# Ladme/groan_rs

Hardware: AMD Instinct MI355X
Metric: frames/sec RMSD-fit, 1e6 atoms triclinic, 1/2/4/8 GPUs; HBM GB/s vs peak (higher is better)
Workload: dtype f32 (fp64 accumulators)

## Files before the change

### groan_rs_amd/csrc/gr_api.hip

```cpp
#include <hip/hip_runtime.h>

#include <cmath>
#include <cstdio>
#include <cstdlib>
#include <cstring>
#include <map>
#include <string>
#include <vector>

#include "../../include/groan_hip.h"
#include "gr_container.h"
#include "gr_kernels.h"
#include "gr_hot.h"
#include "gr_resident.h"
#include "gr_small.h"
#include "gr_xtc.h"
#include "gr_shape.h"
#include "gr_xtc_dev.h"
#include "gr_xtc_enc_dev.h"
#include "gr_trr.h"
#include "gr_cellgrid.h"
#include "gr_textio.h"
#include "gr_pool.h"
#include <set>
// ... 76 lines not shown
    struct Metro { uint64_t shape = 0; double free_ns = 0, T_ns = 0, best_ns = 0, fail_ns = 0; uint32_t off_for = 0, held = 0; } metro;
    uint64_t res_metro_period_ns = 0, res_last_turn_ns = 0, res_late_permille = 0, res_sclk_mhz = 0;
    int wall_khz = 100000;
    uint32_t res_max_wgs = 0;
    int res_test_no_start = 0;
    uint32_t res_test_abort_at = 0xFFFFFFFFu;
    uint32_t res_skip = 0, res_backoff = 0;
    uint32_t *res_progress = nullptr;
    unsigned long long *res_wgrec = nullptr; size_t res_wgrec_cap = 0;
    unsigned long long *res_rec = nullptr;
    uint32_t *res_abort = nullptr;
    uint32_t *res_words_host = nullptr;
    struct ResOut { GrFrameState st[GR_MAX_BATCH]; uint32_t words[16]; alignas(64) uint32_t seq; };
    ResOut *res_out = nullptr, *res_out_dev = nullptr;
    uint32_t res_seq = 0;
    uint32_t res_checkin = 0, res_closed = 0;
    uint32_t res_late_seen[2] = { 0, 0 };
    uint64_t res_lean_segments = 0, res_sync_fallbacks = 0;
    GrShapeSet *shape_set_dev = nullptr;
    unsigned long long *shape_mask_dev = nullptr, *shape_mask_host = nullptr; size_t shape_mask_cap = 0;
    uint32_t res_epoch = 0;
    bool res_in_use = false;
    uint64_t res_launches = 0, res_handshake_misses = 0, res_aborts = 0, res_redone_frames = 0;
    GrFrameState *state_dev = nullptr;
    GrFrameState *state_host = nullptr;
    GrFrameState *small_state = nullptr, *small_state_dev = nullptr;
    uint32_t *small_flag = nullptr, *small_flag_dev = nullptr;
    uint32_t small_seq = 0;
    uint32_t small_max = GR_SMALL_MAX_DEFAULT;
    uint64_t small_calls = 0, small_sync_fallbacks = 0;
    uint32_t *bad_dev = nullptr;
    uint32_t *bad_host = nullptr;
    float *pd_out = nullptr; size_t pd_cap = 0;
    hipEvent_t ev0 = nullptr, ev1 = nullptr;
    hipEvent_t pev[6 * GR_MAX_BATCH] = {};
    uint32_t sub_batch = 256;
    uint32_t chunks = 0;
    uint32_t fit_wgs = 0;
    int profile = 0;
    double prof_ms[4] = { 0, 0, 0, 0 };
    uint64_t prof_launches[4] = { 0, 0, 0, 0 };
    uint64_t prof_frames[4] = { 0, 0, 0, 0 };
    uint32_t n_cus = 0;
    unsigned char *xtc_host[2] = { nullptr, nullptr }, *xtc_dev[2] = { nullptr, nullptr }; size_t xtc_host_cap[2] = { 0, 0 }, xtc_dev_cap[2] = { 0, 0 };
    hipEvent_t xtc_ev[2] = { nullptr, nullptr };
    hipEvent_t xtc_unpacked[2] = { nullptr, nullptr };
// ... 237 lines not shown
    int st = busy_check(c); if (st) return st;
    Group g;
    st = group_build(c, std::move(blocks), &g); if (st) return st;
    const bool existed = c->groups.count(name) != 0;
    if (existed) group_release(c, c->groups[name]);
    c->groups[name] = g;
    c->epoch++;
    return existed ? GR_E_GROUP_EXISTS : GR_OK;
}

const Group *find_group(const gr_ctx *c, const char *name) {
    if (!name) return nullptr;
    auto it = c->groups.find(name);
    return it == c->groups.end() ? nullptr : &it->second;
}

int box_check(gr_ctx *c, uint32_t slot) {
    const int st = c->box_status[slot];
    if (st == GR_E_NO_BOX) return fail(c, GR_E_NO_BOX, "simulation box does not exist");
    if (c->strict && !c->boxes_host[slot].ortho) return fail(c, GR_E_NOT_ORTHOGONAL, "simulation box is not orthogonal");
    if (st != GR_OK) return fail(c, st, st == GR_E_ZERO_BOX ? "box length is not positive" : "box too skewed");
    return GR_OK;
}

int slot_check(gr_ctx *c, uint32_t slot, uint32_t n = 1, bool ingest = false) {
    if (!c) return GR_E_INVALID_ARG;
    if ((uint64_t)slot + n > c->n_slots || n == 0) return fail(c, GR_E_INVALID_ARG, "slot out of range");
    if (!ingest) return busy_check(c);
    if (c->in_flight && slot < c->in_flight_s0 + c->in_flight_n && c->in_flight_s0 < slot + n)
        return fail(c, GR_E_INVALID_ARG, "upload into a slot of the batch in flight: call gr_rmsd_batch_end first (or use the other half of the double buffer)");
    return GR_OK;
}

struct SlotUse {
    gr_ctx *c; uint32_t first, n;
    bool quiet = false;
    SlotUse(gr_ctx *ctx, uint32_t first_slot, uint32_t count = 1) : c(ctx), first(first_slot), n(count) {
        for (uint32_t s = first; s < first + n && s < c->n_slots; ++s)
            if (c->upload_pending[s]) { (void)hipStreamWaitEvent(c->stream, c->ev_ready[s], 0); c->upload_pending[s] = 0; }
    }
    ~SlotUse() {
        if (quiet) return;
        const uint64_t gen = ++c->done_gen;
        (void)hipEventRecord(c->ev_done_ring[gen % 64], c->stream);
        for (uint32_t s = first; s < first + n && s < c->n_slots; ++s) c->slot_gen[s] = gen;
    }
};

static hipError_t sync_ingest(gr_ctx *c) {
    hipError_t e = hipStreamSynchronize(c->copy_stream);
    if (e == hipSuccess && c->unpack_stream) e = hipStreamSynchronize(c->unpack_stream);
    return e;
}
void box_fill(gr_ctx *c, uint32_t slot, const float *box9) {
    GrBox &b = c->boxes_host[slot];
    if (!box9) {
        gr_box_setup(nullptr, &b);
        c->box_status[slot] = GR_E_NO_BOX; c->box9_set[slot] = 0;
    } else {
        const int ok = gr_box_setup(box9, &b);
        memcpy(&c->box9_host[9 * (size_t)slot], box9, 9 * sizeof(float));
        c->box9_set[slot] = 1;
        if (!ok) c->box_status[slot] = GR_E_ZERO_BOX;
        else if (b.ncand > GR_MAX_CAND) c->box_status[slot] = GR_E_UNSUPPORTED_BOX;
        else c->box_status[slot] = GR_OK;
    }
}
int set_box(gr_ctx *c, uint32_t slot, const float *box9, hipStream_t on = nullptr) {
    box_fill(c, slot, box9);
    HIPCHK(c, hipMemcpyAsync(c->boxes_dev + slot, &c->boxes_host[slot], sizeof(GrBox), hipMemcpyHostToDevice, on ? on : c->stream));
    return GR_OK;
}

int set_boxes_same(gr_ctx *c, uint32_t first_slot, uint32_t n, const float *box9, hipStream_t on = nullptr) {
    if (n == 0) return GR_OK;
    float keep[9];
    if (box9) memcpy(keep, box9, sizeof keep);
    box_fill(c, first_slot, box9 ? keep : nullptr);
// ... 67 lines not shown

static int res_next_epoch(gr_ctx *c, uint32_t *epoch) {
    if (++c->res_epoch == 0u) {
        HIPCHK(c, hipStreamSynchronize(c->stream));
        if (c->res_wgrec) HIPCHK(c, hipMemset(c->res_wgrec, 0, c->res_wgrec_cap * sizeof(unsigned long long)));
        HIPCHK(c, hipMemset(c->res_rec, 0, (size_t)GR_MAX_BATCH * 16 * sizeof(unsigned long long)));
        HIPCHK(c, hipMemset(c->res_abort + 2, 0, 2 * sizeof(uint32_t)));
        c->res_epoch = 1u;
    }
    *epoch = c->res_epoch;
    return GR_OK;
}
static int res_test_no_start(gr_ctx *c, uint32_t epoch) {
    if (!c->res_test_no_start) return GR_OK;
    const unsigned long long two = 2ull | ((unsigned long long)epoch << 32);
    c->res_test_no_start = 0;
    HIPCHK(c, hipMemcpyAsync(c->res_abort + 2, &two, sizeof two, hipMemcpyHostToDevice, c->stream));
    HIPCHK(c, hipStreamSynchronize(c->stream));
    return GR_OK;
}
template <int MODE>
static int res_close(gr_ctx *c, uint32_t nb, const double *fit_partials, uint32_t nparts, double sum_w, uint32_t epoch, bool fresh, uint32_t *seq) {
    const uint32_t sq = c->res_seq + 1u;
    k_res_close<MODE><<<dim3(nb), dim3(64), 0, c->stream>>>(fit_partials, nparts, sum_w, c->state_dev, c->res_rec, epoch, fresh ? 1u : 0u, c->res_abort, c->res_closed + nb,
                                                        c->res_out_dev->st, c->res_out_dev->words, &c->res_out_dev->seq, sq);
    HIPCHK(c, hipGetLastError());
    c->res_seq = sq; c->res_closed += nb; *seq = sq;
    return GR_OK;
}
static int res_collect(gr_ctx *c, uint32_t seq, uint32_t nb, uint32_t epoch, bool *started) {
    volatile uint32_t *w = &c->res_out->seq;
    const auto t0 = std::chrono::steady_clock::now();
    for (uint32_t spins = 0; *w != seq; ++spins) {
        if ((spins & 1023u) == 1023u && std::chrono::steady_clock::now() - t0 > std::chrono::milliseconds(20)) {
            c->res_sync_fallbacks++;
            HIPCHK(c, hipStreamSynchronize(c->stream));
            if (*w != seq) return fail(c, GR_E_HIP, "the kernel behind the resident pass ended without publishing its results");
            break;
        }
    }
    std::atomic_thread_fence(std::memory_order_acquire);
    memcpy(c->state_host, c->res_out->st, (size_t)nb * sizeof(GrFrameState));
    memcpy(c->res_words_host, c->res_out->words, 12 * sizeof(uint32_t));
    for (int k = 0; k < 2; ++k) { const uint32_t v = c->res_words_host[8 + k]; c->res_words_host[8 + k] = v - c->res_late_seen[k]; c->res_late_seen[k] = v; }
    *started = c->res_words_host[2] == 1u && c->res_words_host[3] == epoch;
    if (!*started || c->res_words_host[0]) HIPCHK(c, hipStreamSynchronize(c->stream));
    return GR_OK;
// ... 227 lines not shown
    for (int k = 0; k < 6; ++k) if (c->xe_dev[k]) (void)hipFree(c->xe_dev[k]);
    for (int k = 0; k < 2; ++k) if (c->xe_host[k]) (void)hipHostFree(c->xe_host[k]);
    if (c->unpack_stream) { (void)hipStreamSynchronize(c->unpack_stream); (void)hipStreamDestroy(c->unpack_stream); }
    for (int k = 0; k < 2; ++k) {
        if (c->xtc_host[k]) (void)hipHostFree(c->xtc_host[k]);
        if (c->xtc_dev[k]) (void)hipFree(c->xtc_dev[k]);
        if (c->xtc_ev[k]) (void)hipEventDestroy(c->xtc_ev[k]);
        if (c->xtc_unpacked[k]) (void)hipEventDestroy(c->xtc_unpacked[k]);
    }
    if (c->wr_host) (void)hipHostFree(c->wr_host);
    if (c->ev0) (void)hipEventDestroy(c->ev0);
    if (c->ev1) (void)hipEventDestroy(c->ev1);
    for (int k = 0; k < 6 * GR_MAX_BATCH; ++k) if (c->pev[k]) (void)hipEventDestroy(c->pev[k]);
    for (hipEvent_t e : c->ev_ready) if (e) (void)hipEventDestroy(e);
    for (int k = 0; k < 64; ++k) if (c->ev_done_ring[k]) (void)hipEventDestroy(c->ev_done_ring[k]);
    if (c->copy_stream) (void)hipStreamDestroy(c->copy_stream);
    if (c->stream) (void)hipStreamDestroy(c->stream);
    delete c;
} catch (...) { }

const char *gr_last_error(const gr_ctx *c) { return c ? c->err.c_str() : "null context"; }
uint64_t gr_last_error_index(const gr_ctx *c) { return c ? c->err_index : 0; }
void gr_last_error_counts(const gr_ctx *c, uint64_t counts[2]) { if (c && counts) { counts[0] = c->counts[0]; counts[1] = c->counts[1]; } }
int gr_ctx_set_strict_orthogonal(gr_ctx *c, int on) { if (!c) return GR_E_INVALID_ARG; c->strict = on ? 1 : 0; return GR_OK; }
uint64_t gr_n_atoms(const gr_ctx *c) { return c ? c->n : 0; }
uint32_t gr_n_slots(const gr_ctx *c) { return c ? c->n_slots : 0; }

int gr_sync(gr_ctx *c) try {
    if (!c) return GR_E_INVALID_ARG;
    HIPCHK(c, sync_ingest(c));
    HIPCHK(c, hipStreamSynchronize(c->stream));
    return GR_OK;
} catch (...) { return gr_abi_guard(); }

int gr_set_masses(gr_ctx *c, const float *masses, uint64_t n) try {
    if (!c || !masses || n != c->n) return c ? fail(c, GR_E_INVALID_ARG, "masses: size mismatch") : GR_E_INVALID_ARG;
    { int st = busy_check(c); if (st) return st; }
    c->masses_host.assign(masses, masses + n);
    c->epoch++;
    HIPCHK(c, hipMemcpyAsync(c->masses, masses, n * sizeof(float), hipMemcpyHostToDevice, c->stream));
    HIPCHK(c, hipStreamSynchronize(c->stream));
    return GR_OK;
} catch (...) { return gr_abi_guard(); }

size_t gr_container_from_indices(const uint64_t *indices, size_t n, uint64_t n_atoms, uint64_t *os, uint64_t *oe) try {
    return grc::store(grc::from_indices(std::vector<uint64_t>(indices, indices + n), n_atoms), os, oe);
} catch (...) { return 0; }
// ... 821 lines not shown
    if (rec_words > c->res_wgrec_cap) {
        if (c->res_wgrec) (void)hipFree(c->res_wgrec);
        c->res_wgrec = nullptr; c->res_wgrec_cap = 0;
        HIPCHK(c, hipMalloc(&c->res_wgrec, rec_words * sizeof(unsigned long long)));
        HIPCHK(c, hipMemsetAsync(c->res_wgrec, 0, rec_words * sizeof(unsigned long long), S));
        c->res_wgrec_cap = rec_words;
    }
    GrResCtl ctl;
    memset(&ctl, 0, sizeof ctl);
    { const int se = res_next_epoch(c, &ctl.epoch); if (se) return se; }
    ctl.wgrec = c->res_wgrec; ctl.rec = c->res_rec; ctl.abort = c->res_abort; ctl.progress = c->res_progress; ctl.n_stream = res_stream; ctl.n_fin = n_fin;
    ctl.checkin_target = c->res_checkin + res_stream + n_fin; ctl.fresh_states = fresh_states ? 1u : 0u;
    ctl.wgs_frame = wgs; ctl.streams = streams; ctl.groups_wg = gwg;
    ctl.team_waves = resident_team_waves(wgs, streams);
    ctl.patience_ticks = (unsigned long long)c->wall_khz * 3000ull; ctl.start_ticks = (unsigned long long)c->wall_khz * 200ull;
    ctl.test_abort_frame = c->res_test_abort_at; c->res_test_abort_at = 0xFFFFFFFFu;
    ctl.metro_t16 = c->res_metro_ns >= 100 ? (uint32_t)std::min<uint64_t>(0xFFFFFFFFull, (uint64_t)c->res_metro_ns * (uint64_t)c->wall_khz * 16ull / 1000000ull) : 0u;
    ctl.metro_lead = (uint32_t)((uint64_t)c->wall_khz * 2000ull / 1000000ull);
    ctl.cen_weighted = weighted ? 1u : 0u; ctl.cen_dim_mask = (uint32_t)dim_mask;
    float *frames = c->frames; size_t stride = c->frame_stride; uint32_t slot0 = s0, nfr = nb, natoms = (uint32_t)c->n;
    const float *masses = c->masses; GrSel sel_arg = csel; const GrBox *boxes = c->boxes_dev; GrPlanDev plan; memset(&plan, 0, sizeof plan);
    GrFrameState *states = c->state_dev; double *fparts = nullptr;
    void *args[] = { &frames, &stride, &slot0, &nfr, &natoms, &masses, &sel_arg, &boxes, &plan, &states, &fparts, &ctl };
    bool ubox = true;
    for (uint32_t f = 1; f < nb && ubox; ++f) ubox = memcmp(&c->boxes_host[s0 + f], &c->boxes_host[s0], sizeof(GrBox)) == 0;
    const bool fit_last = c->res_fit_last ? c->res_fit_last == 2 : (uint64_t)res_stream * 10u >= (uint64_t)c->res_max_wgs * 9u;
    { const int sn = res_test_no_start(c, ctl.epoch); if (sn) return sn; }
    if (hipLaunchKernel(resident_center_fn(ubox, fit_last), dim3(res_stream + n_fin), dim3(GrResShape::LANES), args, GrResShape::LDS_BYTES, S) != hipSuccess) {
        (void)hipGetLastError();
        c->res_max_wgs = 0;
        return GR_OK;
    }
    c->res_checkin += res_stream + n_fin;
    uint32_t seq = 0; bool started = false;
    { const int sc = res_close<1>(c, nb, nullptr, 0u, 1.0, ctl.epoch, fresh_states, &seq); if (sc) return sc; }
    { const int sc = res_collect(c, seq, nb, ctl.epoch, &started); if (sc) return sc; }
    c->res_last_streams = streams;
    if (!started) {
        c->res_handshake_misses++;
        c->res_backoff = c->res_backoff ? std::min<uint32_t>(c->res_backoff * 2u, 1024u) : 4u;
        c->res_skip = c->res_backoff;
        return GR_OK;
    }
    c->res_backoff = 0;
    c->cen_res_launches++;
    if (fresh_states) c->res_lean_segments++;
    ran = true;
#ifdef GR_EXP_STEPTIME
// ... 215 lines not shown
int gr_ctx_stat(const gr_ctx *c, int key, uint64_t *value) {
    if (!c || !value) return GR_E_INVALID_ARG;
    switch (key) {
    case GR_STAT_N_CUS: *value = c->n_cus; return GR_OK;
    case GR_STAT_RES_MAX_WGS: *value = c->res_max_wgs; return GR_OK;
    case GR_STAT_RES_LAST_STREAMS: *value = c->res_last_streams; return GR_OK;
    case GR_STAT_RES_LAUNCHES: *value = c->res_launches; return GR_OK;
    case GR_STAT_RES_HANDSHAKE_MISSES: *value = c->res_handshake_misses; return GR_OK;
    case GR_STAT_RES_ABORTS: *value = c->res_aborts; return GR_OK;
    case GR_STAT_RES_REDONE_FRAMES: *value = c->res_redone_frames; return GR_OK;
    case GR_STAT_RMSD_FAST_FRAMES: *value = c->rmsd_fast_frames; return GR_OK;
    case GR_STAT_RMSD_EXACT_REDOS: *value = c->rmsd_exact_redos; return GR_OK;
    case GR_STAT_XTC_DEVICE_FRAMES: *value = c->xtc_dev_frames; return GR_OK;
    case GR_STAT_SMALL_CALLS: *value = c->small_calls; return GR_OK;
    case GR_STAT_SMALL_SYNC_FALLBACKS: *value = c->small_sync_fallbacks; return GR_OK;
    case GR_STAT_RES_METRO_PERIOD_NS: *value = c->res_metro_period_ns; return GR_OK;
    case GR_STAT_RES_LAST_TURN_NS: *value = c->res_last_turn_ns; return GR_OK;
    case GR_STAT_RES_LATE_PERMILLE: *value = c->res_late_permille; return GR_OK;
    case GR_STAT_RES_SCLK_MHZ: *value = c->res_sclk_mhz; return GR_OK;
    case GR_STAT_CENTER_RES_LAUNCHES: *value = c->cen_res_launches; return GR_OK;
    case GR_STAT_CENTER_RES_REDONE: *value = c->cen_res_redone; return GR_OK;
    case GR_STAT_RES_LEAN_SEGMENTS: *value = c->res_lean_segments; return GR_OK;
    case GR_STAT_RES_SYNC_FALLBACKS: *value = c->res_sync_fallbacks; return GR_OK;
    default: return GR_E_INVALID_ARG;
    }
}
int gr_ctx_set_tuning(gr_ctx *c, int key, int64_t value) try {
    if (!c) return GR_E_INVALID_ARG;
    { int st = busy_check(c); if (st) return st; }
    switch (key) {
    case GR_TUNE_SUB_BATCH: if (value < 1 || value > GR_MAX_BATCH) break; c->sub_batch = (uint32_t)value; return GR_OK;
    case GR_TUNE_CHUNKS: if (value < 0 || value > GR_MAX_CHUNKS) break; c->chunks = (uint32_t)value; return GR_OK;
    case GR_TUNE_FIT_WGS: if (value < 0 || value > 65535) break; c->fit_wgs = (uint32_t)value; return GR_OK;
    case GR_TUNE_FUSE: c->fuse = value ? 1 : 0; return GR_OK;
    case GR_TUNE_SMALL_CALLS: if (value < 0 || value > 65536) break; c->small_max = (uint32_t)value; return GR_OK;
    case GR_TUNE_TWO_PASS: c->two_pass = value ? 1 : 0; return GR_OK;
    case GR_TUNE_RESIDENT: if (value < 0 || value > 2) break; c->resident = value; return GR_OK;
    case GR_TUNE_MASKED_SELECTIONS: if (value != 0 && value != 1) break; c->masked_sel = (int)value; return GR_OK;
    case GR_TUNE_XTC_DEVICE_ENCODE: if (value != 0 && value != 1) break; c->xtc_dev_encode = (int)value; return GR_OK;
    case GR_TUNE_RMSD_FAST: if (value != 0 && value != 1) break; c->rmsd_fast = (int)value; return GR_OK;
    case GR_TUNE_RMSD_FAST_MIN: if (value < 0 || value > 0x7fffffff) break; c->rmsd_fast_min = (uint32_t)value; return GR_OK;
    case GR_TUNE_RMSD_FAST_SIGMAS: if (value < 0 || value > 1000) break; c->rmsd_fast_sigmas = (int)value; return GR_OK;
    case GR_TUNE_PAIRDIST_SYMMETRIC: if (value != 0 && value != 1) break; c->pd_sym = (int)value; return GR_OK;
    case GR_TUNE_RESIDENT_WG_GROUPS: if (value != 0 && (value < 64 || value > GR_RES_GROUPS || value % 64 != 0)) break; c->res_wg_groups = (int)value; return GR_OK;
    case GR_TUNE_RESIDENT_STREAMS: if (value < 0 || value > GR_RES_MAX_STREAMS) break; c->res_streams = (int)value; return GR_OK;
    case GR_TUNE_RESIDENT_METRO_NS: if (value < 0 || value > 1000000 || (value > 1 && value < 100)) break; c->res_metro_ns = (int)value; c->metro = gr_ctx::Metro(); return GR_OK;
// ... 15 lines not shown
    if (small_ok(c, sel)) {
        k_rmsd_small<1><<<dim3(nf), dim3(64), 0, c->stream>>>(c->frames, c->frame_stride, first_slot, c->masses, sel, c->boxes_dev, p->dev, c->state_dev, 1, nullptr, nullptr, 0u);
    } else {
        const uint32_t nch = chunks_for(sel);
        k_rmsd_accum<1><<<dim3(nch, nf), dim3(GR_WG), 0, c->stream>>>(c->frames, c->frame_stride, first_slot, c->masses, sel, c->boxes_dev, p->dev, c->state_dev, c->acc_partials);
        k_rmsd_finalize<1><<<dim3(nf), dim3(GR_WG), 0, c->stream>>>(c->acc_partials, nch, c->frames, c->frame_stride, first_slot, sel, c->boxes_dev, p->dev, c->state_dev);
    }
    if (fit) {
        const uint32_t gx = (uint32_t)std::min<uint64_t>(((c->n >> 2) + GR_WG * 4 - 1) / (GR_WG * 4) + 1, 1024);
        k_fit_pk<false><<<dim3(gx, nf), dim3(GR_WG), 0, c->stream>>>(c->frames, c->frame_stride, first_slot, (uint32_t)c->n, c->boxes_dev, p->dev, c->state_dev, c->masses, sel, nullptr);
    }
    HIPCHK(c, hipGetLastError());
    return GR_OK;
}

static int segment_begin(gr_rmsd_plan *p, uint32_t s0, uint32_t nb, int fit) {
    gr_ctx *c = p->target;
    Pending &q = p->pend;
    q = Pending();
    q.s0 = s0; q.nb = nb; q.fit = fit; q.active = true;
    SlotUse use(c, s0, nb);
    const Group *g = find_group(c, p->group.c_str());
    q.pre.assign(nb, GR_OK); q.pre_idx.assign(nb, 0); q.pre_msg.assign(nb, std::string());
    for (uint32_t f = 0; f < nb; ++f) {
        int s = box_check(c, s0 + f);
        if (s == GR_OK && !g) s = fail(c, GR_E_GROUP_NOT_FOUND, p->group);
        if (s == GR_OK && g->n == 0) s = fail(c, GR_E_EMPTY_GROUP, p->group);
        q.pre[f] = s;
        if (s != GR_OK) { q.pre_msg[f] = c->err; q.pre_idx[f] = c->err_index; }
        q.any_ok = q.any_ok || s == GR_OK;
    }
    if (!q.any_ok) return GR_OK;
    const GrSel sel = make_sel(*g);
    q.sel = sel; q.group_n = g->n; q.has_group = true;
    if (!p->resolved || p->resolved_epoch != c->epoch) {
        p->resolved_epoch = c->epoch;
        bool same = (g->n == p->n_ref);
        if (same) { size_t k = 0; for (uint64_t i : grc::expand(g->blocks)) { const float a = c->masses_host[i], b = p->w_host[k++]; if (!(a == b)) { same = false; break; } } }
        p->dev.w_is_mass = same ? 1u : 0u; p->resolved = true;
        p->span_ok = p->p_span_dev != nullptr && g->masked && g->mask_dev != nullptr && g->blocks == p->ref_blocks;
    }
    q.consistent = (g->n == p->n_ref);
    const bool fast_asked = c->two_pass && c->rmsd_fast && p->dev.w_is_mass != 0 && g->n >= c->rmsd_fast_min && ((!fit && sel.contiguous) || (sel.masked && p->span_ok));
    const bool small = q.consistent && !p->exact && small_ok(c, sel) && !fast_asked;
    if (small && nb == 1) {
        q.small = true; q.small_seq = ++c->small_seq;
        k_rmsd_small<0><<<dim3(1), dim3(64), 0, c->stream>>>(c->frames, c->frame_stride, s0, c->masses, sel, c->boxes_dev, p->dev,
                                                         c->state_dev, 0, c->small_state_dev, c->small_flag_dev, q.small_seq);
        if (fit) k_fit_pk<false><<<dim3(fit_grid(c, 1), 1), dim3(GR_WG), 0, c->stream>>>(c->frames, c->frame_stride, s0, (uint32_t)c->n, c->boxes_dev, p->dev, c->state_dev, c->masses, sel, nullptr);
        p->fit_behind_small = fit != 0;
        HIPCHK(c, hipGetLastError());
        return GR_OK;
    }
// ... 87 lines not shown
                ctl.metro_lead = (uint32_t)((uint64_t)c->wall_khz * 2000ull / 1000000ull);
            }
#ifdef GR_EXP_STEPTIME
            {
                static unsigned long long *dbg_dev = nullptr;
                if (!dbg_dev) (void)hipMalloc(&dbg_dev, (size_t)GR_MAX_CHUNKS * 8 * 4 * sizeof(unsigned long long));
                ctl.dbg = getenv("GR_STEPTIME") ? dbg_dev : nullptr;
                g_steptime_dbg = ctl.dbg;
            }
#endif
#ifdef GR_EXP_TIMELINE
            {
                static unsigned long long *tl_dev = nullptr; static size_t tl_cap = 0;
                if (nb > tl_cap) { if (tl_dev) (void)hipFree(tl_dev); tl_dev = nullptr; tl_cap = 0; if (hipMalloc(&tl_dev, (size_t)nb * 8 * sizeof(unsigned long long)) == hipSuccess) tl_cap = nb; }
                ctl.tl = getenv("GR_TIMELINE") ? tl_dev : nullptr;
                if (ctl.tl) HIPCHK(c, hipMemsetAsync(ctl.tl, 0, (size_t)nb * 8 * sizeof(unsigned long long), S));
                q.tl_dev = ctl.tl;
            }
#endif
            float *frames = c->frames; size_t stride = c->frame_stride; uint32_t slot0 = s0, nfr = nb, natoms = (uint32_t)c->n;
            const float *masses = c->masses; GrSel sel_arg = sel; const GrBox *boxes = c->boxes_dev; GrPlanDev plan = res_msk ? plan_span : p->dev;
            GrFrameState *states = c->state_dev; double *fparts = c->fit_partials;
            void *args[] = { &frames, &stride, &slot0, &nfr, &natoms, &masses, &sel_arg, &boxes, &plan, &states, &fparts, &ctl };
            bool ubox = true;
            for (uint32_t f = 1; f < nb && ubox; ++f) ubox = memcmp(&c->boxes_host[s0 + f], &c->boxes_host[s0], sizeof(GrBox)) == 0;
#ifdef GR_EXP_NO_UBOX
            ubox = false;
#endif
            const bool whole = sel.start == 0 && sel.n == c->n;
            const bool fit_last = c->res_fit_last ? c->res_fit_last == 2 : (uint64_t)res_stream * 10u >= (uint64_t)c->res_max_wgs * 9u;
            const void *fn = resident_fn(p->dev.w_is_mass != 0, ubox, whole, fit_last);
            const uint32_t lanes = GrResShape::LANES, lds = GrResShape::LDS_BYTES;
            st = res_test_no_start(c, ctl.epoch); if (st) return st;
            if (c->profile) EVREC(c, c->pev[0], true, S);
            const hipError_t le = hipLaunchKernel(fn, dim3(res_stream + n_fin), dim3(lanes), args, lds, S);
            if (le == hipSuccess) {
                if (c->profile) EVREC(c, c->pev[1], true, S);
                c->res_checkin += res_stream + n_fin;
                q.res_fresh = states_unset; q.res_epoch = ctl.epoch;
                states_unset = false;
                st = res_close<0>(c, nb, c->fit_partials, res_wgs * GrResShape::WAVES, p->dev.sw, ctl.epoch, q.res_fresh, &q.res_seq); if (st) return st;
                q.resident = true; q.res_stream = res_stream; q.res_streams = res_streams;
                q.rmsd_fast = false;
                c->res_last_streams = res_streams;
            } else {
                (void)hipGetLastError();
                c->res_max_wgs = 0;
                resident_done(c);
// ... 1311 lines not shown
```

### groan_rs_amd/csrc/gr_resident.h

```cpp
#pragma once
#include <type_traits>
#include "gr_hot.h"

struct GrResShape {
    static constexpr int LANES = 512, WAVES = LANES / 64;
#ifndef GR_RES_K
#define GR_RES_K 6
#endif
    static constexpr int K = GR_RES_K;
    static constexpr int R = 8;
    static constexpr int PARK_F4 = K * 3 * LANES;
    static constexpr int WSUM_F = R * WAVES * 32;
#ifdef GR_EXP_TIMELINE
    static constexpr int TL_BYTES = 128 * 4 * 8;
#else
    static constexpr int TL_BYTES = 0;
#endif
    static constexpr int LDS_BYTES = PARK_F4 * 16 + WSUM_F * 4 + R * WAVES * 8 + 3 * R * 4 + 2 * WAVES * 4 + TL_BYTES;
    static constexpr int REC_PER_WAVE = 256 / WAVES, LANES_PER_REC = 64 / REC_PER_WAVE, WORDS_PER_LANE = 32 / LANES_PER_REC;
};
#ifndef GR_RES_SLEEP
#define GR_RES_SLEEP 2
#endif
#ifndef GR_RES_BAL
// ... 925 lines not shown
            unsigned long long *o = reinterpret_cast<unsigned long long *>(ctl.abort + 16) + ((wg_all ? 2u : 0u) + (wave ? 1u : 0u)) * 8u;
            for (int k = 0; k < 8; ++k) o[k] = st_acc[k];
        }
#endif
        if (clk_wave) {
            const unsigned long long dc = (unsigned long long)clock64() - clk_c0, dw = (unsigned long long)wall_clock64() - clk_w0;
            gr_st_agent(ctl.abort + 10, (uint32_t)(dc >> 8)); gr_st_agent(ctl.abort + 11, (uint32_t)(dw >> 8));
        }
    }
#ifdef GR_EXP_TIMELINE
    if (tl_wg && wave == 0 && !bail) {
        for (uint32_t t = (n_turns > 128u ? n_turns - 128u : 0u) + lane; t < n_turns; t += 64u) {
            const size_t f = kf(t);
            ctl.tl[f * 8 + 0] = tls[(t & 127u) * 4u + 0u];
            ctl.tl[f * 8 + 6] = tls[(t & 127u) * 4u + 1u] | (tls[(t & 127u) * 4u + 2u] << 48);
        }
    }
#endif
}

template <int MODE>
__global__ __launch_bounds__(64) void k_res_close(const double *__restrict__ fit_partials, uint32_t nparts, double sum_w, GrFrameState *state,
                                                  const unsigned long long *__restrict__ rec, uint32_t epoch, uint32_t fresh_states, uint32_t *ctl_words,
                                                  uint32_t done_target, GrFrameState *out_states, uint32_t *out_words, uint32_t *out_seq, uint32_t seq) {
    constexpr uint32_t NW = sizeof(GrFrameState) / 4u, W_RMSD = offsetof(GrFrameState, rmsd) / 4u, W_STATUS = offsetof(GrFrameState, status) / 4u;
    static_assert(sizeof(GrFrameState) % 4u == 0 && NW <= 64u, "a frame state is exported by one wave, a word per lane");
    const uint32_t frame = blockIdx.x, lane = threadIdx.x;
    uint32_t *sw = reinterpret_cast<uint32_t *>(state + frame);
    uint32_t w = 0u;
    if (fresh_states && (uint32_t)(gr_ld_agent(rec + (size_t)frame * 16u) >> 32) != epoch) {
        GrFrameState z = {};
        z.err_index = GR_NOIDX; z.status = GR_ST_ABORTED;
        if (lane < NW) { w = reinterpret_cast<const uint32_t *>(&z)[lane]; sw[lane] = w; }
    } else if (lane < NW) w = sw[lane];
    const int status = __shfl((int)w, (int)W_STATUS, 64);
    if (MODE == 0 && status == 0) {
        double s0 = 0.0, s1 = 0.0, s2 = 0.0, s3 = 0.0;
        const double *p = fit_partials + (size_t)frame * nparts;
        uint32_t k = lane;
        for (; k + 192 < nparts; k += 256) { s0 += p[k]; s1 += p[k + 64]; s2 += p[k + 128]; s3 += p[k + 192]; }
        for (; k < nparts; k += 64) s0 += p[k];
        const double s = gr_wave_sum((s0 + s1) + (s2 + s3));
        float r = 0.0f;
        if (lane == 0) { r = (float)sqrt(fmax(s, 0.0) / sum_w); state[frame].rmsd = r; }
        r = __shfl(r, 0, 64);
        if (lane == W_RMSD) w = __float_as_uint(r);
    }
    if (lane < NW) reinterpret_cast<uint32_t *>(out_states + frame)[lane] = w;
    __threadfence_system();
    uint32_t n = 0u;
    if (lane == 0) n = __hip_atomic_fetch_add(ctl_words + 12, 1u, __ATOMIC_ACQ_REL, __HIP_MEMORY_SCOPE_AGENT) + 1u;
    n = (uint32_t)__builtin_amdgcn_readfirstlane((int)n);
    if (n != done_target) return;
    if (lane < 12u) out_words[lane] = gr_ld_agent(ctl_words + lane);
    __threadfence_system();
    if (lane == 0) __hip_atomic_store(out_seq, seq, __ATOMIC_RELEASE, __HIP_MEMORY_SCOPE_SYSTEM);
}
```

### groan_rs_amd/system.py

```python
import ctypes as C
from enum import IntEnum

import numpy as np

from . import _lib
from ._lib import (OK, E_NO_BOX, E_NOT_ORTHOGONAL, E_ZERO_BOX, E_EMPTY_GROUP, E_INCONSISTENT_GROUP,
                   E_NO_POSITION, E_NO_MASS, E_GROUP_NOT_FOUND, E_OUT_OF_RANGE, E_GROUP_EXISTS, E_INVALID_NAME, E_INVALID_BOND)


class Dimension(IntEnum):
    NONE = 0
    X = 1
    Y = 2
    Z = 3
    XY = 4
    XZ = 5
    YZ = 6
    XYZ = 7

    def is_x(self):
        return self in (Dimension.X, Dimension.XY, Dimension.XZ, Dimension.XYZ)

    def is_y(self):
        return self in (Dimension.Y, Dimension.XY, Dimension.YZ, Dimension.XYZ)
# ... 284 lines not shown
        if st == E_INCONSISTENT_GROUP:
            cnt = (C.c_uint64 * 2)()
            self._lib.gr_last_error_counts(self._ctx, cnt)
            raise RMSDError("InconsistentGroup", (msg, int(cnt[0]), int(cnt[1])), st)
        raise DeviceError(self._lib.gr_status_string(st).decode(), msg, st)

    def get_n_atoms(self):
        return self.n_atoms

    def set_masses(self, masses):
        m = np.ascontiguousarray(masses, dtype=np.float32)
        st = self._lib.gr_set_masses(self._ctx, _ptr(m), m.size)
        if st != OK:
            raise DeviceError("set_masses", self._err(st)[1], st)

    TUNE = {"sub_batch": 1, "chunks": 2, "fit_wgs": 3, "fuse": 4, "two_pass": 5, "resident": 6, "resident_groups": 7, "resident_streams": 8, "resident_fill": 9, "pairdist_symmetric": 10, "resident_wg_groups": 11, "rmsd_fast": 12, "rmsd_fast_min": 13, "rmsd_fast_sigmas": 14, "masked_selections": 15, "xtc_device_encode": 16, "small_calls": 17, "resident_metro_ns": 18, "resident_fit_last": 19, "stream_wgs_per_cu": 20, "center_resident": 21, "translate_rows": 22, "test_resident_no_start": 100, "test_resident_abort_at": 101}

    def set_tuning(self, **kw):
        for k, v in kw.items():
            st = self._lib.gr_ctx_set_tuning(self._ctx, self.TUNE[k], int(v))
            if st != OK:
                raise DeviceError("set_tuning", self._err(st)[1], st)

    STAT = {"n_cus": 1, "res_max_wgs": 2, "res_launches": 3, "res_handshake_misses": 4, "res_aborts": 5, "res_redone_frames": 6, "res_last_streams": 7, "rmsd_fast_frames": 8, "rmsd_exact_redos": 9, "xtc_device_frames": 10, "small_calls": 11, "small_sync_fallbacks": 12, "res_metro_period_ns": 13, "res_last_turn_ns": 14, "res_late_permille": 15, "res_sclk_mhz": 16, "center_res_launches": 17, "center_res_redone": 18, "res_lean_segments": 19, "res_sync_fallbacks": 20}

    def stat(self, key):
        v = C.c_uint64(0)
        st = self._lib.gr_ctx_stat(self._ctx, self.STAT[key], C.byref(v))
        if st != OK:
            raise DeviceError("stat", self._err(st)[1], st)
        return int(v.value)

    def set_center_onepass_min(self, min_atoms):
        self._lib.gr_ctx_set_center_onepass_min(self._ctx, int(min_atoms))

    def center_fallbacks(self):
        return int(self._lib.gr_center_fallbacks(self._ctx))

    def set_strict_orthogonal(self, on=True):
        self._strict_flag = bool(on)
        self._lib.gr_ctx_set_strict_orthogonal(self._ctx, int(bool(on)))

    def group_create_from_ranges(self, name, ranges):
        r = np.asarray(list(ranges), dtype=np.uint64).reshape(-1, 2)
        s, e = np.ascontiguousarray(r[:, 0]), np.ascontiguousarray(r[:, 1])
        st = self._lib.gr_group_create_from_ranges(self._ctx, name.encode(), _ptr(s), _ptr(e), r.shape[0])
        if st not in (OK, E_GROUP_EXISTS):
# ... 478 lines not shown
```

### include/groan_hip.h

```cpp
#ifndef GROAN_HIP_H
#define GROAN_HIP_H
#include <stddef.h>
#include <stdint.h>

#ifdef __cplusplus
extern "C" {
#endif

typedef struct gr_ctx gr_ctx;
typedef struct gr_rmsd_plan gr_rmsd_plan;
typedef struct gr_hbond_plan gr_hbond_plan;
typedef struct gr_gridmap gr_gridmap;
typedef struct gr_xtc gr_xtc;

enum {
    GR_OK = 0,
    GR_E_NO_BOX = 1,
    GR_E_NOT_ORTHOGONAL = 2,
    GR_E_ZERO_BOX = 3,
    GR_E_EMPTY_GROUP = 4,
    GR_E_INCONSISTENT_GROUP = 5,
    GR_E_NO_POSITION = 6,
    GR_E_NO_MASS = 7,
    GR_E_GROUP_NOT_FOUND = 8,
// ... 116 lines not shown
int gr_rmsd_fit_batch(gr_rmsd_plan *plan, uint32_t first_slot, uint32_t n_frames,
                      float *rmsd_out, int *status_out);
int gr_rmsd_batch_begin(gr_rmsd_plan *plan, uint32_t first_slot, uint32_t n_frames, int fit);
int gr_rmsd_batch_end(gr_rmsd_plan *plan, float *rmsd_out, int *status_out, float *R_out);
uint32_t gr_rmsd_plan_last_fallbacks(const gr_rmsd_plan *plan);
int gr_rmsd_plan_force_exact(gr_rmsd_plan *plan, int on);
enum { GR_TUNE_SUB_BATCH = 1, GR_TUNE_CHUNKS = 2, GR_TUNE_FIT_WGS = 3, GR_TUNE_FUSE = 4, GR_TUNE_TWO_PASS = 5, GR_TUNE_RESIDENT = 6, GR_TUNE_RESIDENT_GROUPS = 7,
       GR_TUNE_RESIDENT_STREAMS = 8, GR_TUNE_RESIDENT_FILL = 9, GR_TUNE_PAIRDIST_SYMMETRIC = 10, GR_TUNE_RESIDENT_WG_GROUPS = 11,
       GR_TUNE_RMSD_FAST = 12, GR_TUNE_RMSD_FAST_MIN = 13, GR_TUNE_RESIDENT_METRO_NS = 18, GR_TUNE_RESIDENT_FIT_LAST = 19, GR_TUNE_STREAM_WGS_PER_CU = 20, GR_TUNE_CENTER_RESIDENT = 21, GR_TUNE_TRANSLATE_ROWS = 22,
       GR_TUNE_MASKED_SELECTIONS = 15 ,
       GR_TUNE_XTC_DEVICE_ENCODE = 16 ,
       GR_TUNE_RMSD_FAST_SIGMAS = 14 ,
       GR_TUNE_SMALL_CALLS = 17 ,
       GR_TUNE_TEST_RESIDENT_NO_START = 100 ,
       GR_TUNE_TEST_RESIDENT_ABORT_AT = 101  };
int gr_ctx_set_tuning(gr_ctx *ctx, int key, int64_t value);
enum { GR_STAT_N_CUS = 1, GR_STAT_RES_MAX_WGS = 2, GR_STAT_RES_LAUNCHES = 3, GR_STAT_RES_HANDSHAKE_MISSES = 4, GR_STAT_RES_ABORTS = 5, GR_STAT_RES_REDONE_FRAMES = 6, GR_STAT_RES_LAST_STREAMS = 7,
       GR_STAT_RMSD_FAST_FRAMES = 8 ,
       GR_STAT_RMSD_EXACT_REDOS = 9 ,
       GR_STAT_XTC_DEVICE_FRAMES = 10 ,
       GR_STAT_SMALL_CALLS = 11 ,
       GR_STAT_SMALL_SYNC_FALLBACKS = 12 ,
       GR_STAT_RES_METRO_PERIOD_NS = 13, GR_STAT_RES_LAST_TURN_NS = 14, GR_STAT_RES_LATE_PERMILLE = 15, GR_STAT_RES_SCLK_MHZ = 16,
       GR_STAT_CENTER_RES_LAUNCHES = 17, GR_STAT_CENTER_RES_REDONE = 18, GR_STAT_RES_LEAN_SEGMENTS = 19, GR_STAT_RES_SYNC_FALLBACKS = 20 };
int gr_ctx_stat(const gr_ctx *ctx, int key, uint64_t *value);

enum { GR_PARSE_OK = 0, GR_PARSE_FILE_NOT_FOUND, GR_PARSE_LINE_NOT_FOUND, GR_PARSE_LINE, GR_PARSE_ATOM_LINE, GR_PARSE_BOX_LINE,
       GR_PARSE_UNSUPPORTED_BOX, GR_PARSE_INVALID_FLOAT, GR_PARSE_GROUP_NAME, GR_PARSE_INVALID_ATOM_INDEX };
typedef struct gr_structure gr_structure;
int gr_gro_read(const char *path, gr_structure **out, int *detail_code, char *detail, size_t detail_cap);
void gr_structure_free(gr_structure *s);
uint64_t gr_structure_n_atoms(const gr_structure *s);
const char *gr_structure_title(const gr_structure *s);
int gr_structure_box(const gr_structure *s, float box9[9]);
int gr_structure_positions(const gr_structure *s, float *xyz);
int gr_structure_velocities(const gr_structure *s, float *vel);
int gr_structure_atom(const gr_structure *s, uint64_t i, uint64_t *resid, uint64_t *atomid, char resname[8], char atomname[8]);
typedef struct gr_ndx gr_ndx;
int gr_ndx_read(const char *path, uint64_t n_atoms, gr_ndx **out, int *detail_code, char *detail, size_t detail_cap);
void gr_ndx_free(gr_ndx *x);
size_t gr_ndx_n_groups(const gr_ndx *x);
const char *gr_ndx_group_name(const gr_ndx *x, size_t g);
size_t gr_ndx_group_size(const gr_ndx *x, size_t g);
int gr_ndx_group_indices(const gr_ndx *x, size_t g, uint64_t *out);
int gr_ndx_install(const gr_ndx *x, gr_ctx *ctx, size_t *n_invalid_names, size_t *n_duplicate_names);

int gr_group_pairs_within(gr_ctx *ctx, uint32_t slot, const char *group1, const char *group2, float cutoff, uint64_t max_pairs,
// ... 134 lines not shown
```

Baseline: 140,800.

## Cache per-segment box prechecks and export resident frame states in one bulk copy

Adds a host-side cache keyed on a box generation counter, so the per-frame box validity checks and the uniform-box memcmp scan are skipped when the same segment is rerun with unchanged boxes. Reworks the resident close kernel so each wave writes its frame state only to device memory with an agent-scope release. The last wave then copies all states to the host-mapped output in one pass using 128-bit stores, replacing per-frame system-scope fences. This is meant to cut host CPU overhead and many system-wide fences per batch, at the cost of a serial copy done by a single wave and cache invalidation that must track every path that mutates boxes.

```diff
diff --git a/groan_rs_amd/csrc/gr_api.hip b/groan_rs_amd/csrc/gr_api.hip
--- a/groan_rs_amd/csrc/gr_api.hip
+++ b/groan_rs_amd/csrc/gr_api.hip
@@ -122,6 +122,9 @@
     uint32_t res_epoch = 0;
     bool res_in_use = false;
     uint64_t res_launches = 0, res_handshake_misses = 0, res_aborts = 0, res_redone_frames = 0;
+    uint64_t box_gen = 1;
+    struct PreCache { uint64_t gen = 0; uint32_t s0 = 0, nb = 0; bool boxes_ok = false, ubox_known = false, ubox = false; } pre_cache;
+    uint64_t precheck_cache_hits = 0;
     GrFrameState *state_dev = nullptr;
     GrFrameState *state_host = nullptr;
     GrFrameState *small_state = nullptr, *small_state_dev = nullptr;
@@ -405,6 +408,20 @@
     if (st != GR_OK) return fail(c, st, st == GR_E_ZERO_BOX ? "box length is not positive" : "box too skewed");
     return GR_OK;
 }
+static gr_ctx::PreCache &pre_cache_for(gr_ctx *c, uint32_t s0, uint32_t nb) {
+    gr_ctx::PreCache &pc = c->pre_cache;
+    if (pc.gen != c->box_gen || pc.s0 != s0 || pc.nb != nb) { pc = gr_ctx::PreCache(); pc.gen = c->box_gen; pc.s0 = s0; pc.nb = nb; }
+    return pc;
+}
+static bool segment_ubox(gr_ctx *c, uint32_t s0, uint32_t nb) {
+    gr_ctx::PreCache &pc = pre_cache_for(c, s0, nb);
+    if (!pc.ubox_known) {
+        bool ubox = true;
+        for (uint32_t f = 1; f < nb && ubox; ++f) ubox = memcmp(&c->boxes_host[s0 + f], &c->boxes_host[s0], sizeof(GrBox)) == 0;
+        pc.ubox = ubox; pc.ubox_known = true;
+    }
+    return pc.ubox;
+}
 
 int slot_check(gr_ctx *c, uint32_t slot, uint32_t n = 1, bool ingest = false) {
     if (!c) return GR_E_INVALID_ARG;
@@ -437,6 +454,7 @@
 }
 void box_fill(gr_ctx *c, uint32_t slot, const float *box9) {
     GrBox &b = c->boxes_host[slot];
+    c->box_gen++;
     if (!box9) {
         gr_box_setup(nullptr, &b);
         c->box_status[slot] = GR_E_NO_BOX; c->box9_set[slot] = 0;
@@ -550,7 +568,7 @@
 template <int MODE>
 static int res_close(gr_ctx *c, uint32_t nb, const double *fit_partials, uint32_t nparts, double sum_w, uint32_t epoch, bool fresh, uint32_t *seq) {
     const uint32_t sq = c->res_seq + 1u;
-    k_res_close<MODE><<<dim3(nb), dim3(64), 0, c->stream>>>(fit_partials, nparts, sum_w, c->state_dev, c->res_rec, epoch, fresh ? 1u : 0u, c->res_abort, c->res_closed + nb,
+    k_res_close<MODE><<<dim3(nb), dim3(64), 0, c->stream>>>(fit_partials, nparts, sum_w, c->state_dev, c->res_rec, epoch, fresh ? 1u : 0u, c->res_abort, c->res_closed + nb, nb,
                                                         c->res_out_dev->st, c->res_out_dev->words, &c->res_out_dev->seq, sq);
     HIPCHK(c, hipGetLastError());
     c->res_seq = sq; c->res_closed += nb; *seq = sq;
@@ -824,7 +842,7 @@
 const char *gr_last_error(const gr_ctx *c) { return c ? c->err.c_str() : "null context"; }
 uint64_t gr_last_error_index(const gr_ctx *c) { return c ? c->err_index : 0; }
 void gr_last_error_counts(const gr_ctx *c, uint64_t counts[2]) { if (c && counts) { counts[0] = c->counts[0]; counts[1] = c->counts[1]; } }
-int gr_ctx_set_strict_orthogonal(gr_ctx *c, int on) { if (!c) return GR_E_INVALID_ARG; c->strict = on ? 1 : 0; return GR_OK; }
+int gr_ctx_set_strict_orthogonal(gr_ctx *c, int on) { if (!c) return GR_E_INVALID_ARG; c->strict = on ? 1 : 0; c->box_gen++; return GR_OK; }
 uint64_t gr_n_atoms(const gr_ctx *c) { return c ? c->n : 0; }
 uint32_t gr_n_slots(const gr_ctx *c) { return c ? c->n_slots : 0; }
 
@@ -1692,8 +1710,7 @@
     const float *masses = c->masses; GrSel sel_arg = csel; const GrBox *boxes = c->boxes_dev; GrPlanDev plan; memset(&plan, 0, sizeof plan);
     GrFrameState *states = c->state_dev; double *fparts = nullptr;
     void *args[] = { &frames, &stride, &slot0, &nfr, &natoms, &masses, &sel_arg, &boxes, &plan, &states, &fparts, &ctl };
-    bool ubox = true;
-    for (uint32_t f = 1; f < nb && ubox; ++f) ubox = memcmp(&c->boxes_host[s0 + f], &c->boxes_host[s0], sizeof(GrBox)) == 0;
+    const bool ubox = segment_ubox(c, s0, nb);
     const bool fit_last = c->res_fit_last ? c->res_fit_last == 2 : (uint64_t)res_stream * 10u >= (uint64_t)c->res_max_wgs * 9u;
     { const int sn = res_test_no_start(c, ctl.epoch); if (sn) return sn; }
     if (hipLaunchKernel(resident_center_fn(ubox, fit_last), dim3(res_stream + n_fin), dim3(GrResShape::LANES), args, GrResShape::LDS_BYTES, S) != hipSuccess) {
@@ -1955,6 +1972,7 @@
     case GR_STAT_CENTER_RES_REDONE: *value = c->cen_res_redone; return GR_OK;
     case GR_STAT_RES_LEAN_SEGMENTS: *value = c->res_lean_segments; return GR_OK;
     case GR_STAT_RES_SYNC_FALLBACKS: *value = c->res_sync_fallbacks; return GR_OK;
+    case GR_STAT_PRECHECK_CACHE_HITS: *value = c->precheck_cache_hits; return GR_OK;
     default: return GR_E_INVALID_ARG;
     }
 }
@@ -2016,13 +2034,20 @@
     SlotUse use(c, s0, nb);
     const Group *g = find_group(c, p->group.c_str());
     q.pre.assign(nb, GR_OK); q.pre_idx.assign(nb, 0); q.pre_msg.assign(nb, std::string());
-    for (uint32_t f = 0; f < nb; ++f) {
-        int s = box_check(c, s0 + f);
-        if (s == GR_OK && !g) s = fail(c, GR_E_GROUP_NOT_FOUND, p->group);
-        if (s == GR_OK && g->n == 0) s = fail(c, GR_E_EMPTY_GROUP, p->group);
-        q.pre[f] = s;
-        if (s != GR_OK) { q.pre_msg[f] = c->err; q.pre_idx[f] = c->err_index; }
-        q.any_ok = q.any_ok || s == GR_OK;
+    gr_ctx::PreCache &pc = pre_cache_for(c, s0, nb);
+    if (pc.boxes_ok && g && g->n != 0) { q.any_ok = true; c->precheck_cache_hits++; }
+    else {
+        bool boxes_ok = true;
+        for (uint32_t f = 0; f < nb; ++f) {
+            int s = box_check(c, s0 + f);
+            boxes_ok = boxes_ok && s == GR_OK;
+            if (s == GR_OK && !g) s = fail(c, GR_E_GROUP_NOT_FOUND, p->group);
+            if (s == GR_OK && g->n == 0) s = fail(c, GR_E_EMPTY_GROUP, p->group);
+            q.pre[f] = s;
+            if (s != GR_OK) { q.pre_msg[f] = c->err; q.pre_idx[f] = c->err_index; }
+            q.any_ok = q.any_ok || s == GR_OK;
+        }
+        pc.boxes_ok = boxes_ok;
     }
     if (!q.any_ok) return GR_OK;
     const GrSel sel = make_sel(*g);
@@ -2156,8 +2181,7 @@
             const float *masses = c->masses; GrSel sel_arg = sel; const GrBox *boxes = c->boxes_dev; GrPlanDev plan = res_msk ? plan_span : p->dev;
             GrFrameState *states = c->state_dev; double *fparts = c->fit_partials;
             void *args[] = { &frames, &stride, &slot0, &nfr, &natoms, &masses, &sel_arg, &boxes, &plan, &states, &fparts, &ctl };
-            bool ubox = true;
-            for (uint32_t f = 1; f < nb && ubox; ++f) ubox = memcmp(&c->boxes_host[s0 + f], &c->boxes_host[s0], sizeof(GrBox)) == 0;
+            bool ubox = segment_ubox(c, s0, nb);
 #ifdef GR_EXP_NO_UBOX
             ubox = false;
 #endif
diff --git a/groan_rs_amd/csrc/gr_resident.h b/groan_rs_amd/csrc/gr_resident.h
--- a/groan_rs_amd/csrc/gr_resident.h
+++ b/groan_rs_amd/csrc/gr_resident.h
@@ -971,16 +971,16 @@
 template <int MODE>
 __global__ __launch_bounds__(64) void k_res_close(const double *__restrict__ fit_partials, uint32_t nparts, double sum_w, GrFrameState *state,
                                                   const unsigned long long *__restrict__ rec, uint32_t epoch, uint32_t fresh_states, uint32_t *ctl_words,
-                                                  uint32_t done_target, GrFrameState *out_states, uint32_t *out_words, uint32_t *out_seq, uint32_t seq) {
+                                                  uint32_t done_target, uint32_t nb, GrFrameState *out_states, uint32_t *out_words, uint32_t *out_seq, uint32_t seq) {
     constexpr uint32_t NW = sizeof(GrFrameState) / 4u, W_RMSD = offsetof(GrFrameState, rmsd) / 4u, W_STATUS = offsetof(GrFrameState, status) / 4u;
-    static_assert(sizeof(GrFrameState) % 4u == 0 && NW <= 64u, "a frame state is exported by one wave, a word per lane");
+    static_assert(sizeof(GrFrameState) % 8u == 0 && NW <= 64u, "a frame state is closed by one wave, a word per lane, and exported as 64-bit words");
     const uint32_t frame = blockIdx.x, lane = threadIdx.x;
     uint32_t *sw = reinterpret_cast<uint32_t *>(state + frame);
     uint32_t w = 0u;
     if (fresh_states && (uint32_t)(gr_ld_agent(rec + (size_t)frame * 16u) >> 32) != epoch) {
         GrFrameState z = {};
         z.err_index = GR_NOIDX; z.status = GR_ST_ABORTED;
-        if (lane < NW) { w = reinterpret_cast<const uint32_t *>(&z)[lane]; sw[lane] = w; }
+        if (lane < NW) w = reinterpret_cast<const uint32_t *>(&z)[lane];
     } else if (lane < NW) w = sw[lane];
     const int status = __shfl((int)w, (int)W_STATUS, 64);
     if (MODE == 0 && status == 0) {
@@ -991,16 +991,38 @@
         for (; k < nparts; k += 64) s0 += p[k];
         const double s = gr_wave_sum((s0 + s1) + (s2 + s3));
         float r = 0.0f;
-        if (lane == 0) { r = (float)sqrt(fmax(s, 0.0) / sum_w); state[frame].rmsd = r; }
+        if (lane == 0) r = (float)sqrt(fmax(s, 0.0) / sum_w);
         r = __shfl(r, 0, 64);
         if (lane == W_RMSD) w = __float_as_uint(r);
     }
-    if (lane < NW) reinterpret_cast<uint32_t *>(out_states + frame)[lane] = w;
-    __threadfence_system();
+    if (lane < NW) gr_st_agent(sw + lane, w);
+    __builtin_amdgcn_fence(__ATOMIC_RELEASE, "agent");
     uint32_t n = 0u;
     if (lane == 0) n = __hip_atomic_fetch_add(ctl_words + 12, 1u, __ATOMIC_ACQ_REL, __HIP_MEMORY_SCOPE_AGENT) + 1u;
     n = (uint32_t)__builtin_amdgcn_readfirstlane((int)n);
     if (n != done_target) return;
+    __builtin_amdgcn_fence(__ATOMIC_ACQUIRE, "agent");
+    {
+        constexpr uint32_t UNROLL = 16u;
+        const unsigned long long *src = reinterpret_cast<const unsigned long long *>(state);
+        const uint32_t n64 = nb * (NW / 2u), n128 = n64 / 2u;
+        uint4 *dst = reinterpret_cast<uint4 *>(out_states);
+        for (uint32_t base = 0u; base < n128; base += 64u * UNROLL) {
+            unsigned long long a[UNROLL], b[UNROLL];
+#pragma unroll
+            for (uint32_t u = 0; u < UNROLL; ++u) {
+                const uint32_t i = base + u * 64u + lane;
+                a[u] = 0ull; b[u] = 0ull;
+                if (i < n128) { a[u] = gr_ld_agent(src + 2u * (size_t)i); b[u] = gr_ld_agent(src + 2u * (size_t)i + 1u); }
+            }
+#pragma unroll
+            for (uint32_t u = 0; u < UNROLL; ++u) {
+                const uint32_t i = base + u * 64u + lane;
+                if (i < n128) dst[i] = make_uint4((uint32_t)a[u], (uint32_t)(a[u] >> 32), (uint32_t)b[u], (uint32_t)(b[u] >> 32));
+            }
+        }
+        if ((n64 & 1u) && lane == 0) reinterpret_cast<unsigned long long *>(out_states)[n64 - 1u] = gr_ld_agent(src + (n64 - 1u));
+    }
     if (lane < 12u) out_words[lane] = gr_ld_agent(ctl_words + lane);
     __threadfence_system();
     if (lane == 0) __hip_atomic_store(out_seq, seq, __ATOMIC_RELEASE, __HIP_MEMORY_SCOPE_SYSTEM);
diff --git a/groan_rs_amd/system.py b/groan_rs_amd/system.py
--- a/groan_rs_amd/system.py
+++ b/groan_rs_amd/system.py
@@ -330,7 +330,7 @@
             if st != OK:
                 raise DeviceError("set_tuning", self._err(st)[1], st)
 
-    STAT = {"n_cus": 1, "res_max_wgs": 2, "res_launches": 3, "res_handshake_misses": 4, "res_aborts": 5, "res_redone_frames": 6, "res_last_streams": 7, "rmsd_fast_frames": 8, "rmsd_exact_redos": 9, "xtc_device_frames": 10, "small_calls": 11, "small_sync_fallbacks": 12, "res_metro_period_ns": 13, "res_last_turn_ns": 14, "res_late_permille": 15, "res_sclk_mhz": 16, "center_res_launches": 17, "center_res_redone": 18, "res_lean_segments": 19, "res_sync_fallbacks": 20}
+    STAT = {"n_cus": 1, "res_max_wgs": 2, "res_launches": 3, "res_handshake_misses": 4, "res_aborts": 5, "res_redone_frames": 6, "res_last_streams": 7, "rmsd_fast_frames": 8, "rmsd_exact_redos": 9, "xtc_device_frames": 10, "small_calls": 11, "small_sync_fallbacks": 12, "res_metro_period_ns": 13, "res_last_turn_ns": 14, "res_late_permille": 15, "res_sclk_mhz": 16, "center_res_launches": 17, "center_res_redone": 18, "res_lean_segments": 19, "res_sync_fallbacks": 20, "precheck_cache_hits": 21}
 
     def stat(self, key):
         v = C.c_uint64(0)
diff --git a/include/groan_hip.h b/include/groan_hip.h
--- a/include/groan_hip.h
+++ b/include/groan_hip.h
@@ -162,7 +162,7 @@
        GR_STAT_SMALL_CALLS = 11 ,
        GR_STAT_SMALL_SYNC_FALLBACKS = 12 ,
        GR_STAT_RES_METRO_PERIOD_NS = 13, GR_STAT_RES_LAST_TURN_NS = 14, GR_STAT_RES_LATE_PERMILLE = 15, GR_STAT_RES_SCLK_MHZ = 16,
-       GR_STAT_CENTER_RES_LAUNCHES = 17, GR_STAT_CENTER_RES_REDONE = 18, GR_STAT_RES_LEAN_SEGMENTS = 19, GR_STAT_RES_SYNC_FALLBACKS = 20 };
+       GR_STAT_CENTER_RES_LAUNCHES = 17, GR_STAT_CENTER_RES_REDONE = 18, GR_STAT_RES_LEAN_SEGMENTS = 19, GR_STAT_RES_SYNC_FALLBACKS = 20, GR_STAT_PRECHECK_CACHE_HITS = 21 };
 int gr_ctx_stat(const gr_ctx *ctx, int key, uint64_t *value);
 
 enum { GR_PARSE_OK = 0, GR_PARSE_FILE_NOT_FOUND, GR_PARSE_LINE_NOT_FOUND, GR_PARSE_LINE, GR_PARSE_ATOM_LINE, GR_PARSE_BOX_LINE,
```

Result: slower. 139,400 (-1.0%).
